# biointec/columba

Measured on AMD Instinct MI355X. Metric: reads/sec (150bp, k=4 edit, human ref), higher is better.
Workload: dtype u64; 1 GPU; synthetic human-like reference 3000 Mbp (GRCh38 is not available offline), 10000000 x 150 bp reads per GPU, k=4 edit distance, ALL mode, multiple_opt schemes with dynamic selection, dynamic partitioning, in-text switch 4, SA sparseness 4; reads_per_gpu=10000000, read_len=150, k=4, genome_bp=3000000000, index_bytes_hbm=24766778153, parallelism=read-shard x1, occurrences=33415092

## Files before the change

columba_amd/csrc/columba_amd.hip:

```cpp
#include "../../include/columba_amd.h"
#include "host_schemes.hpp"
#include "host_util.hpp"
#include "kernels.hpp"
#include "units.hpp"

#include <chrono>
#include <cstring>
#include <memory>
#include <mutex>
#include <thread>
#include <string>
#include <vector>

using namespace cmb;

static thread_local std::string g_err;
static int fail(int code, const std::string& msg) {
    g_err = msg;
    return code;
}
namespace cmb {
int failWith(int code, const std::string& msg) { return fail(code, msg); }
}
struct cmb_index {
// ... 481 lines not shown
        if (P > cap) return fail(CMB_ERR_OVERFLOW, "output arrays too small");
        for (uint32_t i = 0; i + 2 < P && seeding; i++) seeding[i] = d.seeding[i];
        for (uint32_t i = 0; i < P && weights; i++) weights[i] = d.weights[i];
        for (uint32_t i = 0; i + 1 < P && begins; i++) begins[i] = d.begins[i];
        if (kmer_cutoff) *kmer_cutoff = s->kmerCutOff;
        return CMB_OK;
    } catch (const std::exception& e) {
        return fail(CMB_ERR_INVALID, e.what());
    }
}

struct cmb_batch {
    cmb_index* ix = nullptr;
    uint32_t k = 0, nReads = 0, maxLen = 0, gw = 0;
    uint32_t minLen = 0;
    int metric = 1;
    DevStrategyK hostStrat{};
    bool wide = false;
    bool wideEdit = false;
    bool noSmallMatrix = false;
    DevStrategyKT<MAXP_WIDE> hostStratW{};
    DevBuf<DevStrategyKT<MAXP_WIDE>> stratW;
    DevBuf<PartOutT<MAXP_WIDE>> partsW;
    uint32_t sNumParts = 0, sPartition = 0, sNSchemes = 0, sMaxSearches = 0;
    hipStream_t stream = nullptr;
    DevBuf<uint8_t> reads, seq;
    DevBuf<uint32_t> rec;
    DevBuf<ExactTask> exq;
    DevBuf<uint8_t> psel;
    uint32_t recW = 0;
    DevBuf<uint64_t> offs;
    DevBuf<uint32_t> G;
    DevBuf<uint4> mfull;
    DevBuf<DevStrategyK> strat;
    DevBuf<uint4> bfsQ[2], bfsEv[2], bfsF, bfsC, bfsA;
    DevBuf<uint32_t> bfsCnt;
    DevBuf<unsigned long long> bfsBlockCnt;
    size_t bfsQCap = 0, bfsEvCap = 0, bfsFCap = 0, bfsCCap = 0, bfsACap = 0;
    DevBuf<uint4> nvQ[2];
    DevBuf<uint32_t> nvCnt;
    size_t nvQCap = 0;
    bool hasNaive = false;
    DevBuf<PartOut> parts;
    DevBuf<DfsTask> dfs;
    DevBuf<uint64_t> vW;
    DevBuf<uint4> tbq;
    DevBuf<uint8_t> dpSlab;
    DevBuf<uint32_t> dpList, dpWork;
    DevBuf<uint4> items;
    DevBuf<FMOccRec> fm, fmUniq;
    DevBuf<TextOccRec> text;
    DevBuf<uint4> fout;
    DevBuf<unsigned long long> keysA, keysB;
    DevBuf<uint32_t> fcounts, fsegB, fsegE, frank;
    DevBuf<uint64_t> foffs;
    DevBuf<unsigned long long> fmKeysA, fmKeysB;
    DevBuf<uint32_t> fmIdxA, fmIdxB, fmN;
    DevBuf<uint8_t> sortTmp, scanTmp;
    DevBuf<unsigned long long> vkeysA, vkeysB;
    DevBuf<uint32_t> vcounts, vruns;
    DevBuf<uint4> vsA[2], vsB[2];
    DevBuf<uint32_t> vsC[2], vsN;
    DevBuf<uint32_t> cnt;
    DevBuf<unsigned long long> counters;
    uint32_t nSlots = 0;
    std::vector<uint64_t> hostOffs;
    bool perStrand = false;
    bool wantAln = false;
    DevBuf<uint32_t> foutRead;
    DevBuf<uint16_t> alnOps;
    DevBuf<AlnRec> alnRec;
    uint32_t alnStride = 0;
    PinnedBuf<uint16_t> hAlnOps;
    PinnedBuf<AlnRec> hAlnRec;
    SamBufs samBufs;
    std::vector<uint4> presetItems;
    std::vector<TextOccRec> presetOut;
    std::vector<cmb_batch*> subs;
    std::vector<uint32_t> subBound;
    DevBuf<uint8_t> readsStage;
    DevBuf<uint64_t> offsStage;
    std::vector<uint64_t> hostOffsStage, hostOffsActive;
    PinnedBuf<uint64_t> offsPin[2];
    int pinNext = 0, pinStaged = 0;
    hipStream_t copyStream = nullptr;
    hipEvent_t copyDone = nullptr;
    bool staged = false;
    const char* pendingSeqs = nullptr;
    bool pending = false;
    cmb_batch* parent = nullptr;
    uint32_t subIndex = 0;
    PinnedBuf<cmb_occ> occs;
    PinnedBuf<uint64_t> occOffs;
    uint64_t cnts[CMB_CNT_MAX];
    std::vector<KernelTime> times;
    bool done = false;
    ~cmb_batch() {
        for (cmb_batch* c : subs) delete c;
        if (copyDone) (void)hipEventDestroy(copyDone);
        if (copyStream) (void)hipStreamDestroy(copyStream);
        if (stream) (void)hipStreamDestroy(stream);
    }
};

static int batchCreateOne(cmb_index* idx, const cmb_strategy* st, uint32_t max_distance, const char* seqs,
                          const uint64_t* offs, uint32_t n_reads, cmb_batch** out);
constexpr uint32_t MAX_SUB_READS = 1u << 23;
// ... 780 lines not shown
                    gridLine(verbose, "k_traceback", nTb, tSlots);
                    const bool narrow = b->k <= TBN_MAX_ED && !getenv("CMB_TRACE_WIDE");
                    const uint32_t tLines = traceLines(narrow, vRows(b->maxLen));
                    if (b->vW.n < (size_t)tLines * 8 * tSlots) b->vW.alloc((size_t)tLines * 8 * tSlots);
                    VPlanes vp{b->vW.p, tSlots, tLines};
                    tm.begin();
                    const uint32_t rowMin = b->minLen > 8u ? b->minLen - 8u : 0u;
                    launchTraceback(s, ix->d, narrow, b->offs.p, mf, b->tbq.p, nTb, vp, q, rowMin);
                    tm.end("k_traceback");
                }
            }
            HIPCHK(hipMemcpyAsync(hcnt, b->cnt.p, sizeof(hcnt), hipMemcpyDeviceToHost, s));
            HIPCHK(hipStreamSynchronize(s));
            if (nFmUniq) {
                tm.begin();
                const uint32_t nb = (uint32_t)std::min<size_t>(((size_t)nFmUniq + 255) / 256, 4096);
                hipLaunchKernelGGL(k_fmocc, dim3(nb), dim3(256), 0, s, ix->d, b->fmUniq.p, nFmUniq, q);
                tm.end("k_fmocc");
            }
            HIPCHK(hipGetLastError());
            HIPCHK(hipMemcpyAsync(hcnt, b->cnt.p, sizeof(hcnt), hipMemcpyDeviceToHost, s));
            HIPCHK(hipStreamSynchronize(s));
            if (hcnt[3] & FLAG_TEXT_OVERFLOW) {
                if (attempt >= 3) return fail(CMB_ERR_INTERNAL, "text occurrence queue keeps overflowing");
                b->text.alloc((size_t)hcnt[2] + hcnt[2] / 8 + 1024);
                HIPCHK(hipMemcpy(b->counters.p, keep, sizeof(keep), hipMemcpyHostToDevice));
                uint32_t fl = hcnt[3] & ~(uint32_t)FLAG_TEXT_OVERFLOW;
                HIPCHK(hipMemcpy(b->cnt.p + 3, &fl, sizeof(uint32_t), hipMemcpyHostToDevice));
                continue;
            }
            break;
        }
        uint32_t nText = hcnt[2];
        lap("verify + traceback + fmocc");
        if (preset) {
            if (hcnt[3] & (FLAG_CAPACITY | FLAG_TRACE_RULE)) return fail(CMB_ERR_INTERNAL, "a traceback left the band");
            b->presetOut.resize(nText);
            if (nText) HIPCHK(hipMemcpy(b->presetOut.data(), b->text.p, (size_t)nText * sizeof(TextOccRec), hipMemcpyDeviceToHost));
            unsigned long long hc2[CMB_CNT_MAX];
            HIPCHK(hipMemcpy(hc2, b->counters.p, sizeof(hc2), hipMemcpyDeviceToHost));
            for (int i = 0; i < CMB_CNT_MAX; i++) b->cnts[i] = hc2[i];
            b->done = true;
            return CMB_OK;
        }

        const uint32_t keyLayout = b->metric == CMB_METRIC_HAMMING ? 1u : b->wideEdit ? 2u : 0u;
        const uint32_t groupShift = keyBits(keyLayout).group;
        uint64_t naiveSurvivors = 0;
        if (b->hasNaive && nText) {
            tm.begin();
            const uint32_t nG = 2u * nReads;
            if (nG >= (1u << (64u - groupShift))) return fail(CMB_ERR_UNSUPPORTED, "more than 2^23 reads in a sub-batch with reads matched by naive backtracking");
            growTo(b->keysA, nText), growTo(b->keysB, nText);
            if (b->fcounts.n < (size_t)nG + 1) {
                b->fcounts.alloc((size_t)nG + 1);
                b->foffs.alloc((size_t)nG + 1);
                b->fsegB.alloc((size_t)nG + 1);
                b->fsegE.alloc((size_t)nG + 1);
            }
            growTo(b->frank, nText);
            hipLaunchKernelGGL(k_pack_keys, dim3((nText + 255) / 256), dim3(256), 0, s, b->text.p, nText, b->offs.p, b->k, b->keysA.p,
                               b->cnt.p, 1u, (const uint8_t*)b->psel.p, keyLayout);
            sortKeys(b->sortTmp, b->keysA.p, b->keysB.p, nText, 0, 64, s);
            const int mode = b->metric == CMB_METRIC_HAMMING ? 1 : 2;
            HIPCHK(hipMemsetAsync(b->fcounts.p, 0, ((size_t)nG + 1) * sizeof(uint32_t), s));
            HIPCHK(hipMemsetAsync(b->fsegB.p, 0xFF, ((size_t)nG + 1) * sizeof(uint32_t), s));
            HIPCHK(hipMemsetAsync(b->frank.p, 0xFF, (size_t)nText * sizeof(uint32_t), s));
            hipLaunchKernelGGL(k_filter_segments, dim3((nText + 255) / 256), dim3(256), 0, s, b->keysB.p, nText, b->fsegB.p, b->fsegE.p, groupShift);
            hipLaunchKernelGGL(k_filter_mark, dim3((nG + 255) / 256), dim3(256), 0, s, b->keysB.p, nG, b->k, mode, b->fcounts.p,
                               b->frank.p, b->fsegB.p, b->fsegE.p, keyLayout);
            scanExclusive(b->scanTmp, b->fcounts.p, b->foffs.p, (size_t)nG + 1, s);
            HIPCHK(hipMemcpyAsync(&naiveSurvivors, b->foffs.p + nG, sizeof(uint64_t), hipMemcpyDeviceToHost, s));
            HIPCHK(hipMemcpyAsync(hcnt, b->cnt.p, sizeof(hcnt), hipMemcpyDeviceToHost, s));
            HIPCHK(hipStreamSynchronize(s));
            if (hcnt[3] & FLAG_CAPACITY)
                return fail(CMB_ERR_INTERNAL, "occurrence does not fit the filter key (width / distance range) or a traceback left the band");
            if ((uint64_t)nText + naiveSurvivors >= 0xFFFFFFF0ull) return fail(CMB_ERR_UNSUPPORTED, "too many occurrences in one sub-batch");
            if (b->text.n < (size_t)nText + naiveSurvivors) {
                DevBuf<TextOccRec> bigger;
                bigger.alloc((size_t)nText + naiveSurvivors + 1024);
                HIPCHK(hipMemcpyAsync(bigger.p, b->text.p, (size_t)nText * sizeof(TextOccRec), hipMemcpyDeviceToDevice, s));
                HIPCHK(hipStreamSynchronize(s));
                std::swap(bigger.p, b->text.p);
                std::swap(bigger.n, b->text.n);
            }
            hipLaunchKernelGGL(k_naive_drop, dim3((nText + 255) / 256), dim3(256), 0, s, b->text.p, nText, (const uint8_t*)b->psel.p);
            if (naiveSurvivors)
                hipLaunchKernelGGL(k_naive_keep, dim3((nText + 255) / 256), dim3(256), 0, s, b->keysB.p, nText, b->offs.p, b->k,
                                   b->frank.p, b->foffs.p, b->text.p + nText, keyLayout);
            HIPCHK(hipGetLastError());
            nText += (uint32_t)naiveSurvivors;
            tm.end("k_naive_filter");
        }

        unsigned long long hc[CMB_CNT_MAX];
        HIPCHK(hipMemcpy(hc, b->counters.p, sizeof(hc), hipMemcpyDeviceToHost));
        for (int i = 0; i < CMB_CNT_MAX; i++) b->cnts[i] = hc[i];
        b->cnts[1] += naiveSurvivors;
        const uint32_t nGroups = b->perStrand ? 2u * nReads : nReads;
        if (nGroups > (1u << (64u - groupShift))) return fail(CMB_ERR_UNSUPPORTED, "more filter groups in one sub-batch than the keys number");
        {
            tm.begin();
            growTo(b->keysA, nText), growTo(b->keysB, nText);
            if (b->fcounts.n < (size_t)nGroups + 1) {
                b->fcounts.alloc((size_t)nGroups + 1);
                b->foffs.alloc((size_t)nGroups + 1);
                b->fsegB.alloc((size_t)nGroups + 1);
                b->fsegE.alloc((size_t)nGroups + 1);
            }
            if (nText) {
                hipLaunchKernelGGL(k_pack_keys, dim3((nText + 255) / 256), dim3(256), 0, s, b->text.p, nText, b->offs.p,
                                   b->k, b->keysA.p, b->cnt.p, b->perStrand ? 1u : 0u, (const uint8_t*)nullptr,
                                   keyLayout);
                sortKeys(b->sortTmp, b->keysA.p, b->keysB.p, nText, 0, 64, s);
            }
            const int mode = b->k == 0 ? 0 : (b->metric == CMB_METRIC_HAMMING ? 1 : 2);
            HIPCHK(hipMemsetAsync(b->fcounts.p, 0, ((size_t)nGroups + 1) * sizeof(uint32_t), s));
            HIPCHK(hipMemsetAsync(b->fsegB.p, 0xFF, ((size_t)nGroups + 1) * sizeof(uint32_t), s));
            if (nText)
                hipLaunchKernelGGL(k_filter_segments, dim3((nText + 255) / 256), dim3(256), 0, s, b->keysB.p, nText, b->fsegB.p,
                                   b->fsegE.p, groupShift);
            growTo(b->frank, nText);
            if (nText) HIPCHK(hipMemsetAsync(b->frank.p, 0xFF, (size_t)nText * sizeof(uint32_t), s));
            hipLaunchKernelGGL(k_filter_mark, dim3((nGroups + 255) / 256), dim3(256), 0, s, b->keysB.p, nGroups, b->k, mode,
                               b->fcounts.p, b->frank.p, b->fsegB.p, b->fsegE.p, keyLayout);
            scanExclusive(b->scanTmp, b->fcounts.p, b->foffs.p, (size_t)nGroups + 1, s);
            uint64_t total = 0;
            HIPCHK(hipMemcpyAsync(&total, b->foffs.p + nGroups, sizeof(uint64_t), hipMemcpyDeviceToHost, s));
            HIPCHK(hipMemcpyAsync(hcnt, b->cnt.p, sizeof(hcnt), hipMemcpyDeviceToHost, s));
            HIPCHK(hipStreamSynchronize(s));
            if (hcnt[3] & FLAG_TRACE_RULE)
                return fail(CMB_ERR_INTERNAL, "a traceback read a band-edge bit the narrow trace rows take as implied");
            if (hcnt[3] & FLAG_CAPACITY)
                return fail(CMB_ERR_INTERNAL, "occurrence does not fit the filter key (width / distance range) or a traceback left the band");
            growTo(b->fout, total);
            if (b->wantAln) growTo(b->foutRead, total);
            if (total)
                hipLaunchKernelGGL(k_filter_write, dim3((nText + 255) / 256), dim3(256), 0, s, b->keysB.p, nText, b->offs.p,
                                   b->k, b->frank.p, b->foffs.p, b->fout.p, b->wantAln ? b->foutRead.p : (uint32_t*)nullptr,
                                   b->perStrand ? 1u : 0u, keyLayout);
            HIPCHK(hipGetLastError());
            tm.end("k_filter");
            lap("filter");
            if (b->wantAln) {
                tm.begin();
                b->alnStride = 2u * b->k + 3u;
                if (b->alnRec.n < total) {
                    b->alnRec.alloc((size_t)total + total / 8 + 256);
                    b->alnOps.alloc(b->alnRec.n * std::max<size_t>(b->alnStride, 2u * 7u + 3u));
                }
                if (total) {
                    const uint32_t cSlots = capSlots((uint32_t)std::min<uint64_t>(((total + 255) / 256) * 256, 512u * 1024u));
                    MFull mfc = mf;
                    if (!mfc.p) mfc.nBlk = 0;
                    const CigarJob job{b->offs.p, b->G.p, b->gw, b->maxLen, mfc, b->fout.p, b->foutRead.p, (uint64_t)total, b->alnOps.p, b->alnStride,
                                       b->alnRec.p, b->cnt.p + 3, (b->metric != CMB_METRIC_EDIT || b->k == 0) ? 1u : 0u};
                    launchCigar(ix, s, job, b->metric == CMB_METRIC_EDIT && b->k > CIGAR_BLOCK_WORDS_MAX_ED, b->k <= TBN_MAX_ED && !getenv("CMB_TRACE_WIDE"),
                                vRows(b->maxLen), cSlots, b->vW, b->dpSlab, verbose);
                }
                tm.end("k_cigar");
                HIPCHK(hipGetLastError());
            }
            b->occs.resize(total);
            b->occOffs.resize((size_t)nGroups + 1);
            if (total) HIPCHK(hipMemcpyAsync(b->occs.data(), b->fout.p, (size_t)total * sizeof(cmb_occ), hipMemcpyDeviceToHost, s));
            if (b->wantAln) {
                b->hAlnRec.resize(total);
                b->hAlnOps.resize((size_t)total * b->alnStride);
                if (total) {
                    HIPCHK(hipMemcpyAsync(b->hAlnRec.data(), b->alnRec.p, (size_t)total * sizeof(AlnRec), hipMemcpyDeviceToHost, s));
                    HIPCHK(hipMemcpyAsync(b->hAlnOps.data(), b->alnOps.p, (size_t)total * b->alnStride * sizeof(uint16_t), hipMemcpyDeviceToHost, s));
                }
                HIPCHK(hipMemcpyAsync(hcnt, b->cnt.p, sizeof(hcnt), hipMemcpyDeviceToHost, s));
            }
            HIPCHK(hipMemcpyAsync(b->occOffs.data(), b->foffs.p, ((size_t)nGroups + 1) * sizeof(uint64_t), hipMemcpyDeviceToHost, s));
            HIPCHK(hipStreamSynchronize(s));
            if (b->wantAln && (hcnt[3] & FLAG_CAPACITY))
                return fail(CMB_ERR_INTERNAL, "a CIGAR traceback left the band or an occurrence is not an alignment within its distance");
            lap("results to the host");
            if (verbose) {
                size_t fr = 0, tot = 0;
                (void)hipMemGetInfo(&fr, &tot);
                fprintf(stderr, "[mem] device memory in use: %.1f GB of %.1f GB\n", (tot - fr) / 1e9, tot / 1e9);
            }
        }
        b->done = true;
        return CMB_OK;
    } catch (const std::exception& e) {
        return fail(CMB_ERR_DEVICE, e.what());
    }
}

namespace cmb {
// ... 541 lines not shown
```

columba_amd/csrc/dev_bfs_naive.hpp:

```cpp
#pragma once
#include <type_traits>

namespace cmb {

struct NaiveBufs {
    uint4* Q[2];
    uint32_t qCap;
    uint32_t* nq;
};

__global__ void __launch_bounds__(256)
k_naive_start(DevIndex ix, const uint8_t* __restrict__ psel, const uint64_t* __restrict__ offs, uint32_t tasks,
              uint32_t k, uint32_t hamming, NaiveBufs B, Queues q, uint32_t narrow = 0 ) {
    const uint32_t rs = blockIdx.x * blockDim.x + threadIdx.x;
    bool root = rs < tasks && (psel[rs] & 0x80u) != 0u;
    if (root && hamming && offs[(rs >> 1) + 1] == offs[rs >> 1]) root = false;
    uint32_t total;
    const uint32_t o = waveAppend(&B.nq[0], root ? 1u : 0u, total);
    if (!root) return;
    if (o >= B.qCap) {
        atomicOr(&q.cnt[3], (uint32_t)FLAG_NAIVE_Q);
        return;
    }
    const uint64_t HP0 = (~0ull) << (narrow ? MXN_LEFT : MX_LEFT);
// ... 99 lines not shown
                    }
                }
                kinds |= kd << (4 * (ch - 1));
                nNode += kd & 1u;
                nIt += (kd & 2u) ? width : 0u;
                nFm += (kd >> 2) & 1u;
            }
        }
        const uint32_t want[4] = {nNode, nIt, nFm, 0u};
        uint32_t got[4];
        blockAppend4(&B.nq[pass + 1], &q.cnt[0], &q.cnt[1], &q.cnt[1], want, sh, got);
        uint32_t oNode = got[0], oIt = got[1], oFm = got[2];
        bool ok = true;
        if (oNode + nNode > qCap) { ok = false; flags |= FLAG_NAIVE_Q; }
        if (oIt + nIt > q.itemCap) { ok = false; flags |= FLAG_ITEM_OVERFLOW; }
        if (oFm + nFm > q.fmCap) { ok = false; flags |= FLAG_FMOCC_OVERFLOW; }
        if (ok && kinds) {
            const uint32_t itMeta = EDIT ? packMeta(0u, k, 0u, 1u, ITEM_EDIT) : packMeta(0u, k, 0u, 0u, ITEM_HAMMING);
#pragma unroll
            for (int c = 0; c < 4; c++) {
                const uint32_t kd = (kinds >> (4 * c)) & 15u;
                if (kd & 4u) q.fm[oFm++] = FMOccRec{rsId, cr[c].x, cr[c].y, row1, cDist[c], 0u};
                if (kd & 1u) {
                    const uint32_t racOrV = cr[c].z;
                    Qo[oNode] = make_uint4(cr[c].x, cr[c].y, 0u, 0u);
                    Qo[(size_t)qCap + oNode] = make_uint4(rsId, cState[c], racOrV, 0u);
                    if (EDIT)
                        Qo[(size_t)2 * qCap + oNode] = make_uint4((uint32_t)cHP[c], (uint32_t)(cHP[c] >> 32), (uint32_t)cHN[c],
                                                                  (uint32_t)(cHN[c] >> 32));
                    oNode++;
                } else if (kd & 2u) {
                    const uint32_t w = cr[c].y - cr[c].x;
                    for (uint32_t t = 0; t < w; t++) q.items[oIt + t] = make_uint4(rsId, cr[c].x + t, 0u, itMeta);
                    oIt += w;
                }
            }
        }
    }
    const uint32_t local[3] = {cNode, cExp, cRows};
    const int which[3] = {0, 7, 11};
    flushCounters(q, local, which, 3);
    if (flags) atomicOr(&q.cnt[3], flags);
}

__global__ void __launch_bounds__(256)
k_naive_drop(TextOccRec* __restrict__ text, uint32_t n, const uint8_t* __restrict__ psel) {
    const uint32_t i = blockIdx.x * blockDim.x + threadIdx.x;
    if (i >= n) return;
    const uint32_t rs = text[i].rsId;
    if (rs != 0xFFFFFFFFu && (psel[rs] & 0x80u)) text[i].rsId = 0xFFFFFFFFu;
}
__global__ void __launch_bounds__(256)
k_naive_keep(const unsigned long long* __restrict__ keys, uint32_t n, const uint64_t* __restrict__ offs, uint32_t k,
             const uint32_t* __restrict__ rank, const uint64_t* __restrict__ outOffs, TextOccRec* __restrict__ out, uint32_t layout) {
    const KeyBits kb = keyBits(layout);
    const uint32_t i = blockIdx.x * blockDim.x + threadIdx.x;
    if (i >= n) return;
    const uint32_t rk = rank[i];
    if (rk == 0xFFFFFFFFu) return;
    const unsigned long long key = keys[i];
    const uint32_t rs = (uint32_t)(key >> kb.group), r = rs >> 1;
    const uint32_t len = (uint32_t)(offs[r + 1] - offs[r]);
    const uint32_t begin = (uint32_t)(key >> kb.begin), dist = (uint32_t)(key >> kb.dist) & kb.distMask;
    const uint32_t width = layout == 1u ? len : len - k + ((uint32_t)(key >> 1) & kb.wMask);
    out[outOffs[rs] + rk] = TextOccRec{rs, begin, begin + width, dist};
}

}
```

columba_amd/csrc/kernels.hpp:

```cpp
#pragma once
#include "dev_partition.hpp"
#include "host_util.hpp"
#include <cstring>
#include <rocprim/device/device_radix_sort.hpp>
#include <rocprim/device/device_scan.hpp>
#include <rocprim/device/device_run_length_encode.hpp>

namespace cmb {

__global__ void k_rank(DevIndex ix, int rev, const uint32_t* __restrict__ c, const uint64_t* __restrict__ p,
                       uint64_t n, uint64_t* __restrict__ out) {
    const uint64_t i = (uint64_t)blockIdx.x * blockDim.x + threadIdx.x;
    if (i >= n) return;
    out[i] = rank1(rev ? ix.rev : ix.fwd, c[i], p[i]);
}

__device__ __forceinline__ uint32_t rank9RefLayout(const uint64_t* bv, const uint64_t* cnt, uint64_t nWords, uint64_t p) {
    uint64_t w = p >> 6, b = p & 63;
    if (nWords == 0) return 0;
    if (w >= nWords) {
        w = nWords - 1;
        b = 64;
    }
    uint64_t rv = cnt[(w >> 3) * 2];
// ... 1733 lines not shown
                    if (t + j >= w) break;
                    cLF += sa[j] & (ix.saSparseness - 1u);
                    const uint32_t p = sa[j] + f.shift;
                    q.text[o + t + j] = TextOccRec{f.rsId, p, p + f.depth, f.dist};
                }
            }
            cLoc += w;
            continue;
        }
        for (uint32_t t = 0; t < w; t++) {
            cLoc++;
            const uint32_t p = findSA(ix, f.b + t, &cLF) + f.shift;
            q.text[o + t] = TextOccRec{f.rsId, p, p + f.depth, f.dist};
        }
    }
    const uint32_t local[2] = {cLF, cLoc};
    const int which[2] = {8, 9};
    flushCounters(q, local, which, 2);
    if (flags) atomicOr(&q.cnt[3], flags);
}

__global__ void __launch_bounds__(256)
k_pack_keys(const TextOccRec* __restrict__ text, uint32_t n, const uint64_t* __restrict__ offs, uint32_t k,
            unsigned long long* __restrict__ keys, uint32_t* __restrict__ cnt,
            uint32_t perStrand ,
            const uint8_t* __restrict__ only = nullptr ,
            uint32_t layout = 0 ) {
    const uint32_t i = blockIdx.x * blockDim.x + threadIdx.x;
    if (i >= n) return;
    const TextOccRec t = text[i];
    if (t.rsId == 0xFFFFFFFFu || (only && !(only[t.rsId] & 0x80u))) {
        keys[i] = ~0ull;
        return;
    }
    const uint32_t r = t.rsId >> 1;
    const uint32_t len = (uint32_t)(offs[r + 1] - offs[r]);
    const uint32_t width = t.end - t.begin;
    const uint32_t wrel = width - (len - k);
    const uint32_t grp = perStrand ? t.rsId : r;
    const KeyBits kb = keyBits(layout);
    uint32_t low;
    if (layout == 1u) {
        if (width != len || t.dist > kb.distMask) atomicOr(&cnt[3], (uint32_t)FLAG_CAPACITY);
        low = (t.dist & kb.distMask) << kb.dist;
    } else {
        if (wrel > kb.wMask || t.dist > kb.distMask) atomicOr(&cnt[3], (uint32_t)FLAG_CAPACITY);
        low = ((t.dist & kb.distMask) << kb.dist) | ((wrel & kb.wMask) << 1);
    }
    if ((unsigned long long)grp >> (64u - kb.group)) atomicOr(&cnt[3], (uint32_t)FLAG_CAPACITY);
    keys[i] = ((unsigned long long)grp << kb.group) | ((unsigned long long)t.begin << kb.begin) | (unsigned long long)low |
              (unsigned long long)(perStrand ? 0u : (t.rsId & 1u));
}

__global__ void k_filter_segments(const unsigned long long* __restrict__ keys, uint32_t n, uint32_t* __restrict__ segBeg,
                                  uint32_t* __restrict__ segEnd, uint32_t groupShift = 40u) {
    const uint32_t i = blockIdx.x * blockDim.x + threadIdx.x;
    if (i >= n) return;
    const unsigned long long key = keys[i];
    if (key == ~0ull) return;
    const uint32_t r = (uint32_t)(key >> groupShift);
    if (i == 0 || (uint32_t)(keys[i - 1] >> groupShift) != r) segBeg[r] = i;
    if (i + 1 == n || keys[i + 1] == ~0ull || (uint32_t)(keys[i + 1] >> groupShift) != r) segEnd[r] = i + 1;
}

constexpr uint32_t FILTER_NONE = 0xFFFFFFFFu;
constexpr uint32_t FILTER_SHORT = 24;
__global__ void __launch_bounds__(256)
k_filter_mark(const unsigned long long* __restrict__ keys, uint32_t nReads, uint32_t k, int mode,
              uint32_t* __restrict__ counts, uint32_t* __restrict__ rank, const uint32_t* __restrict__ segBeg,
              const uint32_t* __restrict__ segEnd, uint32_t layout = 0u) {
    const KeyBits kb = keyBits(layout);
    const uint32_t r = blockIdx.x * blockDim.x + threadIdx.x;
    const uint32_t lane = threadIdx.x & 63u;
    uint32_t segLo = 0xFFFFFFFFu;
    if (r < nReads) segLo = segBeg[r];
    const bool has = segLo != 0xFFFFFFFFu;
    const uint32_t nSeg = has ? segEnd[r] - segLo : 0u;
    const uint32_t maxDiff = 2 * k;
    struct State {
        uint32_t nOut = 0, lastKept = 0, prevBegin = 0xFFFFFFFFu, prevDepth = 0xFFFFFFFFu, prevED;
        unsigned long long prevKey = ~0ull;
    };
    auto stepCore = [&](State& st, uint32_t i, unsigned long long key, uint32_t& replaced) -> uint32_t {
        const uint32_t begin = (uint32_t)(key >> kb.begin), dist = (uint32_t)(key >> kb.dist) & kb.distMask;
        const uint32_t width = (uint32_t)(key >> 1) & kb.wMask;
        replaced = FILTER_NONE;
        bool keep = true;
        if (mode != 0) {
            if ((key >> 1) == (st.prevKey >> 1)) keep = false;
            else st.prevKey = key;
        }
        if (keep && mode == 2) {
            const uint32_t diff = begin > st.prevBegin ? begin - st.prevBegin : st.prevBegin - begin;
            if (diff == 0) keep = false;
            else if (diff <= maxDiff) {
                if (dist > st.prevED || (dist == st.prevED && width >= st.prevDepth)) keep = false;
                else {
                    st.nOut--;
                    replaced = st.lastKept;
                }
            }
            if (keep) {
                st.prevBegin = begin;
                st.prevED = dist;
                st.prevDepth = width;
            }
        }
        uint32_t mine = FILTER_NONE;
        if (keep) {
            mine = st.nOut++;
            st.lastKept = i;
        }
        return mine;
    };
    State mySt;
    mySt.prevED = k + 1;
    auto step = [&](uint32_t i, unsigned long long key) {
        uint32_t replaced;
        const uint32_t mine = stepCore(mySt, i, key, replaced);
        if (replaced != FILTER_NONE) rank[segLo + replaced] = FILTER_NONE;
        rank[segLo + i] = mine;
    };
    const bool isShort = nSeg <= FILTER_SHORT;
    if (has && isShort) {
        unsigned long long first[8];
#pragma unroll
        for (uint32_t j = 0; j < 8; j++) first[j] = j < nSeg ? keys[segLo + j] : 0ull;
#pragma unroll
        for (uint32_t j = 0; j < 8; j++)
            if (j < nSeg) step(j, first[j]);
        if (nSeg > 8u) {
            unsigned long long nxt[FILTER_SHORT - 8];
#pragma unroll
            for (uint32_t j = 0; j < FILTER_SHORT - 8; j++) nxt[j] = 8u + j < nSeg ? keys[segLo + 8u + j] : 0ull;
#pragma unroll
            for (uint32_t j = 0; j < FILTER_SHORT - 8; j++)
                if (8u + j < nSeg) step(8u + j, nxt[j]);
        }
    }
    unsigned long long todo = __ballot(has && !isShort);
    while (todo) {
        const int owner = __ffsll((long long)todo) - 1;
        todo &= todo - 1ull;
        const uint32_t oLo = (uint32_t)__builtin_amdgcn_readlane((int)segLo, owner);
        const uint32_t oN = (uint32_t)__builtin_amdgcn_readlane((int)nSeg, owner);
        State u;
        u.prevED = k + 1;
        unsigned long long nextKey = lane < oN ? keys[oLo + lane] : 0ull;
        for (uint32_t base = 0; base < oN; base += 64u) {
            const unsigned long long mineKey = nextKey;
            if (base + 64u < oN) nextKey = base + 64u + lane < oN ? keys[oLo + base + 64u + lane] : 0ull;
            const uint32_t cnt = min(64u, oN - base);
            uint32_t myRank = FILTER_NONE;
            for (uint32_t j = 0; j < cnt; j++) {
                const uint32_t lo = (uint32_t)__builtin_amdgcn_readlane((int)(uint32_t)mineKey, (int)j);
                const uint32_t hi = (uint32_t)__builtin_amdgcn_readlane((int)(uint32_t)(mineKey >> 32), (int)j);
                uint32_t replaced;
                const uint32_t mine = stepCore(u, base + j, (unsigned long long)lo | ((unsigned long long)hi << 32), replaced);
                if (replaced != FILTER_NONE) {
                    if (replaced >= base) {
                        if (lane == replaced - base) myRank = FILTER_NONE;
                    } else if (lane == (replaced & 63u)) {
                        rank[oLo + replaced] = FILTER_NONE;
                    }
                }
                if (lane == j) myRank = mine;
            }
            if (lane < cnt) rank[oLo + base + lane] = myRank;
        }
        if (lane == (uint32_t)owner) mySt.nOut = u.nOut;
    }
    const uint32_t nOut = mySt.nOut;
    if (r < nReads) counts[r] = nOut;
}
__global__ void __launch_bounds__(256)
k_filter_write(const unsigned long long* __restrict__ keys, uint32_t n, const uint64_t* __restrict__ offs, uint32_t k,
               const uint32_t* __restrict__ rank, const uint64_t* __restrict__ outOffs, uint4* __restrict__ out,
               uint32_t* __restrict__ outRead , uint32_t perStrand, uint32_t layout) {
    const KeyBits kb = keyBits(layout);
    const uint32_t i = blockIdx.x * blockDim.x + threadIdx.x;
    if (i >= n) return;
    const uint32_t rk = rank[i];
    if (rk == FILTER_NONE) return;
    const unsigned long long key = keys[i];
    const uint32_t grp = (uint32_t)(key >> kb.group);
    const uint32_t r = perStrand ? grp >> 1 : grp;
    const uint32_t len = (uint32_t)(offs[r + 1] - offs[r]);
    const uint32_t begin = (uint32_t)(key >> kb.begin), dist = (uint32_t)(key >> kb.dist) & kb.distMask;
    const uint32_t width = layout == 1u ? len : len - k + ((uint32_t)(key >> 1) & kb.wMask), strand = perStrand ? (grp & 1u) : ((uint32_t)key & 1u);
    out[outOffs[grp] + rk] = make_uint4(begin, begin + width, dist, strand);
    if (outRead) outRead[outOffs[grp] + rk] = r;
}

constexpr uint32_t CIG_M = 0, CIG_I = 1, CIG_D = 2;
constexpr uint32_t CIGAR_BLOCK_WORDS_MAX_ED = 9;
template <bool NARROW, bool PACKED>
__global__ void __launch_bounds__(256)
k_cigar(DevIndex ix, const uint64_t* __restrict__ offs, MFull mf, const uint4* __restrict__ occs,
        const uint32_t* __restrict__ occRead, uint64_t nOcc, VPlanes V, const uint32_t* __restrict__ seqStarts, uint32_t nSeqs,
        uint16_t* __restrict__ ops, uint32_t stride, AlnRec* __restrict__ aln, uint32_t* __restrict__ flagWord,
        uint32_t gapless ) {
    __shared__ uint64_t wW[NARROW ? 1 : TBW][256];
    __shared__ uint32_t wN[NARROW ? 16 : 1][256];
    __shared__ uint64_t Ml[ML_WORDS];
    const uint32_t slot = blockIdx.x * blockDim.x + threadIdx.x;
    const uint32_t tid = threadIdx.x;
    uint32_t flags = 0, dummyRows = 0;
    const uint64_t strideT = (uint64_t)gridDim.x * blockDim.x;
    const uint64_t HP0 = (~0ull) << MXW_LEFT;
    for (uint64_t base = slot & ~63u; base < nOcc; base += strideT) {
        const uint64_t it = base + (tid & 63u);
        uint4 o = make_uint4(0, 0, 0, 0);
        uint32_t rs = 0, len = 0, size = 0, col = 0;
        bool have = false;
        if (it < nOcc) {
            o = occs[it];
            rs = 2u * occRead[it] + (o.w & 1u);
            len = (uint32_t)(offs[(rs >> 1) + 1] - offs[rs >> 1]);
            size = o.y - o.x;
            have = true;
            uint32_t lo = 0, hi = nSeqs;
            while (hi - lo > 1) {
                const uint32_t mid = (lo + hi) >> 1;
                if (seqStarts[mid] <= o.x) lo = mid;
                else hi = mid;
            }
            aln[it].seqId = lo;
            aln[it].seqBegin = o.x - seqStarts[lo];
            aln[it].spans = o.y > seqStarts[lo + 1] ? 1u : 0u;
        }
        const uint32_t maxED = o.z;
        MatGeom g;
        g.n = len + 1;
        g.maxED = maxED;
        g.Wv = maxED;
        g.Wh = maxED;
        g.m = max(g.Wv + g.n, g.Wv + g.Wh + 1u);
        col = len;
        bool trace = have && maxED > 0 && size > 0 && !gapless;
        if (trace && NARROW && maxED > TBN_MAX_ED) {
            flags |= FLAG_CAPACITY;
            trace = false;
        }
        uint32_t dummyMask;
// ... 210 lines not shown
```

Before: 64.50 million reads/s.

## Parallelise occurrence filter per key instead of per read group

Replaces the per-read-group filter (segment detection, per-group walk, per-group count scan) with a per-occurrence keep flag. Only cluster heads, meaning keys more than 2k apart from their predecessor, walk their short cluster, and long clusters fall back to wave-cooperative processing. A scan over keep flags then gives output positions, and group offsets are rebuilt inside the write kernel with a wave fill. This removes the segment kernel, several memsets and the load imbalance from very uneven groups, at the cost of a scan over all occurrences rather than over groups.

```diff
diff --git a/columba_amd/csrc/columba_amd.hip b/columba_amd/csrc/columba_amd.hip
--- a/columba_amd/csrc/columba_amd.hip
+++ b/columba_amd/csrc/columba_amd.hip
@@ -557,7 +557,7 @@
     DevBuf<TextOccRec> text;
     DevBuf<uint4> fout;
     DevBuf<unsigned long long> keysA, keysB;
-    DevBuf<uint32_t> fcounts, fsegB, fsegE, frank;
+    DevBuf<uint32_t> fkeep, fpos;
     DevBuf<uint64_t> foffs;
     DevBuf<unsigned long long> fmKeysA, fmKeysB;
     DevBuf<uint32_t> fmIdxA, fmIdxB, fmN;
@@ -1444,27 +1444,18 @@
             const uint32_t nG = 2u * nReads;
             if (nG >= (1u << (64u - groupShift))) return fail(CMB_ERR_UNSUPPORTED, "more than 2^23 reads in a sub-batch with reads matched by naive backtracking");
             growTo(b->keysA, nText), growTo(b->keysB, nText);
-            if (b->fcounts.n < (size_t)nG + 1) {
-                b->fcounts.alloc((size_t)nG + 1);
-                b->foffs.alloc((size_t)nG + 1);
-                b->fsegB.alloc((size_t)nG + 1);
-                b->fsegE.alloc((size_t)nG + 1);
-            }
-            growTo(b->frank, nText);
+            growTo(b->fkeep, (size_t)nText + 1), growTo(b->fpos, (size_t)nText + 1);
             hipLaunchKernelGGL(k_pack_keys, dim3((nText + 255) / 256), dim3(256), 0, s, b->text.p, nText, b->offs.p, b->k, b->keysA.p,
                                b->cnt.p, 1u, (const uint8_t*)b->psel.p, keyLayout);
             sortKeys(b->sortTmp, b->keysA.p, b->keysB.p, nText, 0, 64, s);
             const int mode = b->metric == CMB_METRIC_HAMMING ? 1 : 2;
-            HIPCHK(hipMemsetAsync(b->fcounts.p, 0, ((size_t)nG + 1) * sizeof(uint32_t), s));
-            HIPCHK(hipMemsetAsync(b->fsegB.p, 0xFF, ((size_t)nG + 1) * sizeof(uint32_t), s));
-            HIPCHK(hipMemsetAsync(b->frank.p, 0xFF, (size_t)nText * sizeof(uint32_t), s));
-            hipLaunchKernelGGL(k_filter_segments, dim3((nText + 255) / 256), dim3(256), 0, s, b->keysB.p, nText, b->fsegB.p, b->fsegE.p, groupShift);
-            hipLaunchKernelGGL(k_filter_mark, dim3((nG + 255) / 256), dim3(256), 0, s, b->keysB.p, nG, b->k, mode, b->fcounts.p,
-                               b->frank.p, b->fsegB.p, b->fsegE.p, keyLayout);
-            scanExclusive(b->scanTmp, b->fcounts.p, b->foffs.p, (size_t)nG + 1, s);
-            HIPCHK(hipMemcpyAsync(&naiveSurvivors, b->foffs.p + nG, sizeof(uint64_t), hipMemcpyDeviceToHost, s));
+            hipLaunchKernelGGL(k_filter_mark, dim3(nText / 256 + 1), dim3(256), 0, s, b->keysB.p, nText, b->k, mode, b->fkeep.p, keyLayout);
+            scanExclusive(b->scanTmp, b->fkeep.p, b->fpos.p, (size_t)nText + 1, s);
+            uint32_t kept = 0;
+            HIPCHK(hipMemcpyAsync(&kept, b->fpos.p + nText, sizeof(uint32_t), hipMemcpyDeviceToHost, s));
             HIPCHK(hipMemcpyAsync(hcnt, b->cnt.p, sizeof(hcnt), hipMemcpyDeviceToHost, s));
             HIPCHK(hipStreamSynchronize(s));
+            naiveSurvivors = kept;
             if (hcnt[3] & FLAG_CAPACITY)
                 return fail(CMB_ERR_INTERNAL, "occurrence does not fit the filter key (width / distance range) or a traceback left the band");
             if ((uint64_t)nText + naiveSurvivors >= 0xFFFFFFF0ull) return fail(CMB_ERR_UNSUPPORTED, "too many occurrences in one sub-batch");
@@ -1479,7 +1470,7 @@
             hipLaunchKernelGGL(k_naive_drop, dim3((nText + 255) / 256), dim3(256), 0, s, b->text.p, nText, (const uint8_t*)b->psel.p);
             if (naiveSurvivors)
                 hipLaunchKernelGGL(k_naive_keep, dim3((nText + 255) / 256), dim3(256), 0, s, b->keysB.p, nText, b->offs.p, b->k,
-                                   b->frank.p, b->foffs.p, b->text.p + nText, keyLayout);
+                                   b->fkeep.p, b->fpos.p, b->text.p + nText, keyLayout);
             HIPCHK(hipGetLastError());
             nText += (uint32_t)naiveSurvivors;
             tm.end("k_naive_filter");
@@ -1494,43 +1485,34 @@
         {
             tm.begin();
             growTo(b->keysA, nText), growTo(b->keysB, nText);
-            if (b->fcounts.n < (size_t)nGroups + 1) {
-                b->fcounts.alloc((size_t)nGroups + 1);
-                b->foffs.alloc((size_t)nGroups + 1);
-                b->fsegB.alloc((size_t)nGroups + 1);
-                b->fsegE.alloc((size_t)nGroups + 1);
-            }
+            growTo(b->fkeep, (size_t)nText + 1), growTo(b->fpos, (size_t)nText + 1);
+            if (b->foffs.n < (size_t)nGroups + 1) b->foffs.alloc((size_t)nGroups + 1);
+            const int mode = b->k == 0 ? 0 : (b->metric == CMB_METRIC_HAMMING ? 1 : 2);
+            uint32_t kept = 0;
             if (nText) {
                 hipLaunchKernelGGL(k_pack_keys, dim3((nText + 255) / 256), dim3(256), 0, s, b->text.p, nText, b->offs.p,
                                    b->k, b->keysA.p, b->cnt.p, b->perStrand ? 1u : 0u, (const uint8_t*)nullptr,
                                    keyLayout);
                 sortKeys(b->sortTmp, b->keysA.p, b->keysB.p, nText, 0, 64, s);
+                hipLaunchKernelGGL(k_filter_mark, dim3(nText / 256 + 1), dim3(256), 0, s, b->keysB.p, nText, b->k, mode, b->fkeep.p, keyLayout);
+                scanExclusive(b->scanTmp, b->fkeep.p, b->fpos.p, (size_t)nText + 1, s);
+                HIPCHK(hipMemcpyAsync(&kept, b->fpos.p + nText, sizeof(uint32_t), hipMemcpyDeviceToHost, s));
+            } else {
+                HIPCHK(hipMemsetAsync(b->foffs.p, 0, ((size_t)nGroups + 1) * sizeof(uint64_t), s));
             }
-            const int mode = b->k == 0 ? 0 : (b->metric == CMB_METRIC_HAMMING ? 1 : 2);
-            HIPCHK(hipMemsetAsync(b->fcounts.p, 0, ((size_t)nGroups + 1) * sizeof(uint32_t), s));
-            HIPCHK(hipMemsetAsync(b->fsegB.p, 0xFF, ((size_t)nGroups + 1) * sizeof(uint32_t), s));
-            if (nText)
-                hipLaunchKernelGGL(k_filter_segments, dim3((nText + 255) / 256), dim3(256), 0, s, b->keysB.p, nText, b->fsegB.p,
-                                   b->fsegE.p, groupShift);
-            growTo(b->frank, nText);
-            if (nText) HIPCHK(hipMemsetAsync(b->frank.p, 0xFF, (size_t)nText * sizeof(uint32_t), s));
-            hipLaunchKernelGGL(k_filter_mark, dim3((nGroups + 255) / 256), dim3(256), 0, s, b->keysB.p, nGroups, b->k, mode,
-                               b->fcounts.p, b->frank.p, b->fsegB.p, b->fsegE.p, keyLayout);
-            scanExclusive(b->scanTmp, b->fcounts.p, b->foffs.p, (size_t)nGroups + 1, s);
-            uint64_t total = 0;
-            HIPCHK(hipMemcpyAsync(&total, b->foffs.p + nGroups, sizeof(uint64_t), hipMemcpyDeviceToHost, s));
             HIPCHK(hipMemcpyAsync(hcnt, b->cnt.p, sizeof(hcnt), hipMemcpyDeviceToHost, s));
             HIPCHK(hipStreamSynchronize(s));
+            const uint64_t total = kept;
             if (hcnt[3] & FLAG_TRACE_RULE)
                 return fail(CMB_ERR_INTERNAL, "a traceback read a band-edge bit the narrow trace rows take as implied");
             if (hcnt[3] & FLAG_CAPACITY)
                 return fail(CMB_ERR_INTERNAL, "occurrence does not fit the filter key (width / distance range) or a traceback left the band");
             growTo(b->fout, total);
             if (b->wantAln) growTo(b->foutRead, total);
-            if (total)
+            if (nText)
                 hipLaunchKernelGGL(k_filter_write, dim3((nText + 255) / 256), dim3(256), 0, s, b->keysB.p, nText, b->offs.p,
-                                   b->k, b->frank.p, b->foffs.p, b->fout.p, b->wantAln ? b->foutRead.p : (uint32_t*)nullptr,
-                                   b->perStrand ? 1u : 0u, keyLayout);
+                                   b->k, b->fkeep.p, b->fpos.p, nGroups, b->foffs.p, b->fout.p,
+                                   b->wantAln ? b->foutRead.p : (uint32_t*)nullptr, b->perStrand ? 1u : 0u, keyLayout);
             HIPCHK(hipGetLastError());
             tm.end("k_filter");
             lap("filter");
diff --git a/columba_amd/csrc/dev_bfs_naive.hpp b/columba_amd/csrc/dev_bfs_naive.hpp
--- a/columba_amd/csrc/dev_bfs_naive.hpp
+++ b/columba_amd/csrc/dev_bfs_naive.hpp
@@ -175,18 +175,17 @@
 }
 __global__ void __launch_bounds__(256)
 k_naive_keep(const unsigned long long* __restrict__ keys, uint32_t n, const uint64_t* __restrict__ offs, uint32_t k,
-             const uint32_t* __restrict__ rank, const uint64_t* __restrict__ outOffs, TextOccRec* __restrict__ out, uint32_t layout) {
+             const uint32_t* __restrict__ keep, const uint32_t* __restrict__ pos ,
+             TextOccRec* __restrict__ out, uint32_t layout) {
     const KeyBits kb = keyBits(layout);
     const uint32_t i = blockIdx.x * blockDim.x + threadIdx.x;
-    if (i >= n) return;
-    const uint32_t rk = rank[i];
-    if (rk == 0xFFFFFFFFu) return;
+    if (i >= n || !keep[i]) return;
     const unsigned long long key = keys[i];
     const uint32_t rs = (uint32_t)(key >> kb.group), r = rs >> 1;
     const uint32_t len = (uint32_t)(offs[r + 1] - offs[r]);
     const uint32_t begin = (uint32_t)(key >> kb.begin), dist = (uint32_t)(key >> kb.dist) & kb.distMask;
     const uint32_t width = layout == 1u ? len : len - k + ((uint32_t)(key >> 1) & kb.wMask);
-    out[outOffs[rs] + rk] = TextOccRec{rs, begin, begin + width, dist};
+    out[pos[i]] = TextOccRec{rs, begin, begin + width, dist};
 }
 
 }
diff --git a/columba_amd/csrc/kernels.hpp b/columba_amd/csrc/kernels.hpp
--- a/columba_amd/csrc/kernels.hpp
+++ b/columba_amd/csrc/kernels.hpp
@@ -1809,144 +1809,170 @@
               (unsigned long long)(perStrand ? 0u : (t.rsId & 1u));
 }
 
-__global__ void k_filter_segments(const unsigned long long* __restrict__ keys, uint32_t n, uint32_t* __restrict__ segBeg,
-                                  uint32_t* __restrict__ segEnd, uint32_t groupShift = 40u) {
+constexpr uint32_t FILTER_NONE = 0xFFFFFFFFu;
+constexpr uint32_t FILTER_WALK = 16;
+struct FilterState {
+    uint32_t lastKept = 0, prevBegin = 0xFFFFFFFFu, prevDepth = 0xFFFFFFFFu, prevED = 0;
+    unsigned long long prevKey = ~0ull;
+};
+__device__ __forceinline__ bool filterStep(FilterState& st, const KeyBits kb, uint32_t maxDiff, uint32_t i, unsigned long long key,
+                                           uint32_t& replaced) {
+    const uint32_t begin = (uint32_t)(key >> kb.begin), dist = (uint32_t)(key >> kb.dist) & kb.distMask;
+    const uint32_t width = (uint32_t)(key >> 1) & kb.wMask;
+    replaced = FILTER_NONE;
+    if ((key >> 1) == (st.prevKey >> 1)) return false;
+    st.prevKey = key;
+    const uint32_t diff = begin > st.prevBegin ? begin - st.prevBegin : st.prevBegin - begin;
+    if (diff == 0) return false;
+    if (diff <= maxDiff) {
+        if (dist > st.prevED || (dist == st.prevED && width >= st.prevDepth)) return false;
+        replaced = st.lastKept;
+    }
+    st.prevBegin = begin;
+    st.prevED = dist;
+    st.prevDepth = width;
+    st.lastKept = i;
+    return true;
+}
+__global__ void __launch_bounds__(256)
+k_filter_mark(const unsigned long long* __restrict__ keys, uint32_t n, uint32_t k, int mode, uint32_t* __restrict__ keep ,
+              uint32_t layout = 0u) {
+    const KeyBits kb = keyBits(layout);
     const uint32_t i = blockIdx.x * blockDim.x + threadIdx.x;
-    if (i >= n) return;
-    const unsigned long long key = keys[i];
-    if (key == ~0ull) return;
-    const uint32_t r = (uint32_t)(key >> groupShift);
-    if (i == 0 || (uint32_t)(keys[i - 1] >> groupShift) != r) segBeg[r] = i;
-    if (i + 1 == n || keys[i + 1] == ~0ull || (uint32_t)(keys[i + 1] >> groupShift) != r) segEnd[r] = i + 1;
-}
-
-constexpr uint32_t FILTER_NONE = 0xFFFFFFFFu;
-constexpr uint32_t FILTER_SHORT = 24;
-__global__ void __launch_bounds__(256)
-k_filter_mark(const unsigned long long* __restrict__ keys, uint32_t nReads, uint32_t k, int mode,
-              uint32_t* __restrict__ counts, uint32_t* __restrict__ rank, const uint32_t* __restrict__ segBeg,
-              const uint32_t* __restrict__ segEnd, uint32_t layout = 0u) {
-    const KeyBits kb = keyBits(layout);
-    const uint32_t r = blockIdx.x * blockDim.x + threadIdx.x;
     const uint32_t lane = threadIdx.x & 63u;
-    uint32_t segLo = 0xFFFFFFFFu;
-    if (r < nReads) segLo = segBeg[r];
-    const bool has = segLo != 0xFFFFFFFFu;
-    const uint32_t nSeg = has ? segEnd[r] - segLo : 0u;
     const uint32_t maxDiff = 2 * k;
-    struct State {
-        uint32_t nOut = 0, lastKept = 0, prevBegin = 0xFFFFFFFFu, prevDepth = 0xFFFFFFFFu, prevED;
-        unsigned long long prevKey = ~0ull;
-    };
-    auto stepCore = [&](State& st, uint32_t i, unsigned long long key, uint32_t& replaced) -> uint32_t {
-        const uint32_t begin = (uint32_t)(key >> kb.begin), dist = (uint32_t)(key >> kb.dist) & kb.distMask;
-        const uint32_t width = (uint32_t)(key >> 1) & kb.wMask;
-        replaced = FILTER_NONE;
-        bool keep = true;
-        if (mode != 0) {
-            if ((key >> 1) == (st.prevKey >> 1)) keep = false;
-            else st.prevKey = key;
-        }
-        if (keep && mode == 2) {
-            const uint32_t diff = begin > st.prevBegin ? begin - st.prevBegin : st.prevBegin - begin;
-            if (diff == 0) keep = false;
-            else if (diff <= maxDiff) {
-                if (dist > st.prevED || (dist == st.prevED && width >= st.prevDepth)) keep = false;
-                else {
-                    st.nOut--;
-                    replaced = st.lastKept;
-                }
-            }
-            if (keep) {
-                st.prevBegin = begin;
-                st.prevED = dist;
-                st.prevDepth = width;
-            }
-        }
-        uint32_t mine = FILTER_NONE;
-        if (keep) {
-            mine = st.nOut++;
-            st.lastKept = i;
-        }
-        return mine;
-    };
-    State mySt;
-    mySt.prevED = k + 1;
-    auto step = [&](uint32_t i, unsigned long long key) {
-        uint32_t replaced;
-        const uint32_t mine = stepCore(mySt, i, key, replaced);
-        if (replaced != FILTER_NONE) rank[segLo + replaced] = FILTER_NONE;
-        rank[segLo + i] = mine;
-    };
-    const bool isShort = nSeg <= FILTER_SHORT;
-    if (has && isShort) {
-        unsigned long long first[8];
-#pragma unroll
-        for (uint32_t j = 0; j < 8; j++) first[j] = j < nSeg ? keys[segLo + j] : 0ull;
-#pragma unroll
-        for (uint32_t j = 0; j < 8; j++)
-            if (j < nSeg) step(j, first[j]);
-        if (nSeg > 8u) {
-            unsigned long long nxt[FILTER_SHORT - 8];
-#pragma unroll
-            for (uint32_t j = 0; j < FILTER_SHORT - 8; j++) nxt[j] = 8u + j < nSeg ? keys[segLo + 8u + j] : 0ull;
-#pragma unroll
-            for (uint32_t j = 0; j < FILTER_SHORT - 8; j++)
-                if (8u + j < nSeg) step(8u + j, nxt[j]);
-        }
-    }
-    unsigned long long todo = __ballot(has && !isShort);
+    const unsigned long long key = i < n ? keys[i] : ~0ull;
+    const bool real = key != ~0ull;
+    const uint32_t grp = (uint32_t)(key >> kb.group);
+    if (i <= n && (!real || mode == 0)) keep[i] = real ? 1u : 0u;
+    bool head = false;
+    FilterState st;
+    st.prevED = k + 1;
+    if (real && mode != 0) {
+        const unsigned long long prev = i ? keys[i - 1] : ~0ull;
+        const bool groupHead = i == 0 || (uint32_t)(prev >> kb.group) != grp;
+        if (mode == 1) keep[i] = (groupHead || (key >> 1) != (prev >> 1)) ? 1u : 0u;
+        else {
+            head = groupHead || (uint32_t)(key >> kb.begin) - (uint32_t)(prev >> kb.begin) > maxDiff;
+            if (!groupHead) {
+                st.prevKey = prev;
+                st.prevBegin = (uint32_t)(prev >> kb.begin);
+            }
+        }
+    }
+    uint32_t j = 0;
+    uint32_t lastBegin = (uint32_t)(key >> kb.begin);
+    bool more = head;
+    if (head) {
+        auto step = [&](unsigned long long x) {
+            uint32_t replaced;
+            const bool kept = filterStep(st, kb, maxDiff, j, x, replaced);
+            if (replaced != FILTER_NONE) keep[i + replaced] = 0u;
+            keep[i + j] = kept ? 1u : 0u;
+            lastBegin = (uint32_t)(x >> kb.begin);
+            j++;
+        };
+        step(key);
+        while (more && j < FILTER_WALK) {
+            unsigned long long c[4];
+#pragma unroll
+            for (uint32_t t = 0; t < 4; t++) c[t] = (uint64_t)i + j + t < n ? keys[i + j + t] : ~0ull;
+#pragma unroll
+            for (uint32_t t = 0; t < 4; t++) {
+                if (!more) break;
+                if (c[t] == ~0ull || (uint32_t)(c[t] >> kb.group) != grp || (uint32_t)(c[t] >> kb.begin) - lastBegin > maxDiff) more = false;
+                else step(c[t]);
+            }
+        }
+    }
+    auto bcast = [](uint32_t v, int from) { return (uint32_t)__builtin_amdgcn_readlane((int)v, from); };
+    unsigned long long todo = __ballot(head && more);
     while (todo) {
         const int owner = __ffsll((long long)todo) - 1;
         todo &= todo - 1ull;
-        const uint32_t oLo = (uint32_t)__builtin_amdgcn_readlane((int)segLo, owner);
-        const uint32_t oN = (uint32_t)__builtin_amdgcn_readlane((int)nSeg, owner);
-        State u;
-        u.prevED = k + 1;
-        unsigned long long nextKey = lane < oN ? keys[oLo + lane] : 0ull;
-        for (uint32_t base = 0; base < oN; base += 64u) {
+        const uint32_t oI = bcast(i, owner), oJ = bcast(j, owner), oGrp = bcast(grp, owner);
+        uint32_t uBegin = bcast(lastBegin, owner);
+        FilterState u;
+        u.lastKept = bcast(st.lastKept, owner), u.prevBegin = bcast(st.prevBegin, owner), u.prevDepth = bcast(st.prevDepth, owner);
+        u.prevED = bcast(st.prevED, owner);
+        u.prevKey = (unsigned long long)bcast((uint32_t)st.prevKey, owner) | ((unsigned long long)bcast((uint32_t)(st.prevKey >> 32), owner) << 32);
+        const uint64_t start = (uint64_t)oI + oJ;
+        unsigned long long nextKey = start + lane < n ? keys[start + lane] : ~0ull;
+        bool on = true;
+        for (uint32_t base = 0; on; base += 64u) {
             const unsigned long long mineKey = nextKey;
-            if (base + 64u < oN) nextKey = base + 64u + lane < oN ? keys[oLo + base + 64u + lane] : 0ull;
-            const uint32_t cnt = min(64u, oN - base);
-            uint32_t myRank = FILTER_NONE;
-            for (uint32_t j = 0; j < cnt; j++) {
-                const uint32_t lo = (uint32_t)__builtin_amdgcn_readlane((int)(uint32_t)mineKey, (int)j);
-                const uint32_t hi = (uint32_t)__builtin_amdgcn_readlane((int)(uint32_t)(mineKey >> 32), (int)j);
+            nextKey = start + base + 64u + lane < n ? keys[start + base + 64u + lane] : ~0ull;
+            uint32_t myKeep = 0u, cnt = 0u;
+            for (uint32_t t = 0; t < 64u; t++) {
+                const unsigned long long x = (unsigned long long)bcast((uint32_t)mineKey, (int)t) | ((unsigned long long)bcast((uint32_t)(mineKey >> 32), (int)t) << 32);
+                const uint32_t xBegin = (uint32_t)(x >> kb.begin);
+                if (x == ~0ull || (uint32_t)(x >> kb.group) != oGrp || xBegin - uBegin > maxDiff) {
+                    on = false;
+                    break;
+                }
+                const uint32_t num = oJ + base + t;
                 uint32_t replaced;
-                const uint32_t mine = stepCore(u, base + j, (unsigned long long)lo | ((unsigned long long)hi << 32), replaced);
+                const bool kept = filterStep(u, kb, maxDiff, num, x, replaced);
                 if (replaced != FILTER_NONE) {
-                    if (replaced >= base) {
-                        if (lane == replaced - base) myRank = FILTER_NONE;
-                    } else if (lane == (replaced & 63u)) {
-                        rank[oLo + replaced] = FILTER_NONE;
-                    }
-                }
-                if (lane == j) myRank = mine;
-            }
-            if (lane < cnt) rank[oLo + base + lane] = myRank;
-        }
-        if (lane == (uint32_t)owner) mySt.nOut = u.nOut;
-    }
-    const uint32_t nOut = mySt.nOut;
-    if (r < nReads) counts[r] = nOut;
+                    if (replaced >= oJ + base) {
+                        if (lane == replaced - (oJ + base)) myKeep = 0u;
+                    } else if (replaced >= oJ) {
+                        if (lane == ((replaced - oJ) & 63u)) keep[oI + replaced] = 0u;
+                    } else if (lane == (uint32_t)owner) {
+                        keep[oI + replaced] = 0u;
+                    }
+                }
+                if (lane == t) myKeep = kept ? 1u : 0u;
+                uBegin = xBegin;
+                cnt = t + 1u;
+            }
+            if (lane < cnt) keep[start + base + lane] = myKeep;
+        }
+    }
+}
+__device__ __forceinline__ void waveFill(uint64_t* __restrict__ a, uint32_t lo, uint32_t hi, uint64_t v) {
+    const uint32_t lane = threadIdx.x & 63u;
+    const bool far = hi > lo && hi - lo > 4u;
+    if (!far)
+        for (uint32_t g = lo; g < hi; g++) a[g] = v;
+    unsigned long long todo = __ballot(far);
+    while (todo) {
+        const int owner = __ffsll((long long)todo) - 1;
+        todo &= todo - 1ull;
+        const uint32_t oLo = (uint32_t)__builtin_amdgcn_readlane((int)lo, owner), oHi = (uint32_t)__builtin_amdgcn_readlane((int)hi, owner);
+        const uint32_t vLo = (uint32_t)__builtin_amdgcn_readlane((int)(uint32_t)v, owner);
+        const uint32_t vHi = (uint32_t)__builtin_amdgcn_readlane((int)(uint32_t)(v >> 32), owner);
+        for (uint64_t g = (uint64_t)oLo + lane; g < oHi; g += 64u) a[g] = (uint64_t)vLo | ((uint64_t)vHi << 32);
+    }
 }
 __global__ void __launch_bounds__(256)
 k_filter_write(const unsigned long long* __restrict__ keys, uint32_t n, const uint64_t* __restrict__ offs, uint32_t k,
-               const uint32_t* __restrict__ rank, const uint64_t* __restrict__ outOffs, uint4* __restrict__ out,
+               const uint32_t* __restrict__ keep, const uint32_t* __restrict__ pos , uint32_t nGroups,
+               uint64_t* __restrict__ groupOffs , uint4* __restrict__ out,
                uint32_t* __restrict__ outRead , uint32_t perStrand, uint32_t layout) {
     const KeyBits kb = keyBits(layout);
     const uint32_t i = blockIdx.x * blockDim.x + threadIdx.x;
-    if (i >= n) return;
-    const uint32_t rk = rank[i];
-    if (rk == FILTER_NONE) return;
-    const unsigned long long key = keys[i];
+    const unsigned long long key = i < n ? keys[i] : ~0ull;
+    const bool real = key != ~0ull;
     const uint32_t grp = (uint32_t)(key >> kb.group);
+    uint32_t lo = 0, hi = 0, tailLo = 0, tailHi = 0, p = 0, total = 0;
+    if (real) {
+        p = pos[i];
+        const uint32_t before = i ? (uint32_t)(keys[i - 1] >> kb.group) + 1u : 0u;
+        if (before <= grp) lo = before, hi = grp + 1u;
+        if (i + 1 == n || keys[i + 1] == ~0ull) tailLo = grp + 1u, tailHi = nGroups + 1u, total = pos[i + 1];
+    } else if (i == 0) {
+        tailHi = nGroups + 1u;
+    }
+    waveFill(groupOffs, lo, hi, p);
+    waveFill(groupOffs, tailLo, tailHi, total);
+    if (!real || !keep[i]) return;
     const uint32_t r = perStrand ? grp >> 1 : grp;
     const uint32_t len = (uint32_t)(offs[r + 1] - offs[r]);
     const uint32_t begin = (uint32_t)(key >> kb.begin), dist = (uint32_t)(key >> kb.dist) & kb.distMask;
     const uint32_t width = layout == 1u ? len : len - k + ((uint32_t)(key >> 1) & kb.wMask), strand = perStrand ? (grp & 1u) : ((uint32_t)key & 1u);
-    out[outOffs[grp] + rk] = make_uint4(begin, begin + width, dist, strand);
-    if (outRead) outRead[outOffs[grp] + rk] = r;
+    out[p] = make_uint4(begin, begin + width, dist, strand);
+    if (outRead) outRead[p] = r;
 }
 
 constexpr uint32_t CIG_M = 0, CIG_I = 1, CIG_D = 2;
```

Result: no change. 64.08 million reads/s (-0.7%).
